# TencentARC/HOSNeRF

Hardware: AMD Instinct MI355X
Metric: train rays/sec (stage3: forward + losses + backward + gradient all-reduce + Adam; LPIPS term OFF in this line -- stages.stage3_with_lpips carries it) (higher is better)
Workload: dtype f32 (fp16/bf16 hi-lo split MFMA x3, fp32 accumulate)

## Files before the change

hosnerf_amd/csrc/hos_compact.hip:

```cpp
#include "hos_common.h"

namespace {

constexpr int CT = 256;
constexpr int CPT = 4;
constexpr int CB = CT * CPT;
constexpr int CMAXB = 4096;

__global__ __launch_bounds__(CT) void compact_count_kernel(const float* mask, float thr, long P, int* blk_off, unsigned int* ticket,
                                                          int* count) {
    __shared__ int sh[CT / 64];
    __shared__ bool last;
    const int tid = threadIdx.x;
    const long base = (long)blockIdx.x * CB + tid * CPT;
    int c = 0;
#pragma unroll
    for (int k = 0; k < CPT; ++k) c += (base + k < P && mask[base + k] > thr) ? 1 : 0;
    for (int o = 32; o > 0; o >>= 1) c += __shfl_xor(c, o, 64);
    if ((tid & 63) == 0) sh[tid >> 6] = c;
    __syncthreads();
    if (tid == 0) {
        int tot = 0;
        for (int w = 0; w < CT / 64; ++w) tot += sh[w];
        blk_off[blockIdx.x] = tot;
// ... 95 lines not shown
__global__ __launch_bounds__(LT) void live_scan_kernel(const int* __restrict__ flag, int B, int S, int* __restrict__ ray_ids,
                                                       int* __restrict__ rows_live) {
    __shared__ int wsum[LT / 64];
    __shared__ int total;
    const int t = threadIdx.x, lane = t & 63, wave = t >> 6;
    const int per = (B + LT - 1) / LT;
    const int r0 = t * per;
    int c = 0;
    for (int k = 0; k < per; ++k) c += (r0 + k < B && flag[r0 + k] != 0) ? 1 : 0;
    int incl = c;
    for (int o = 1; o < 64; o <<= 1) { const int n = __shfl_up(incl, o, 64); if (lane >= o) incl += n; }
    if (lane == 63) wsum[wave] = incl;
    __syncthreads();
    int pos = incl - c;
    for (int w = 0; w < wave; ++w) pos += wsum[w];
    if (t == LT - 1) { total = pos + c; *rows_live = (pos + c) * S; }
    for (int k = 0; k < per; ++k)
        if (r0 + k < B && flag[r0 + k] != 0) ray_ids[pos++] = r0 + k;
    __syncthreads();
    const int n = total;
    for (int i = n + t; i < B; i += LT) ray_ids[i] = -1;
}

__global__ __launch_bounds__(256) void gather_rays_kernel(const float* __restrict__ src, const int* __restrict__ ray_ids,
                                                         const int* __restrict__ rows_live, long P, int S, int C, float* __restrict__ dst) {
    const long total = P * C;
    const long live = min((long)*rows_live, P) * C;
    for (long i = (long)blockIdx.x * blockDim.x + threadIdx.x; i < total; i += (long)gridDim.x * blockDim.x) {
        float v = 0.f;
        if (i < live) {
            const long j = i / C;
            const int c = (int)(i - j * C);
            const long ray = ray_ids[j / S];
            v = src[(ray * S + j % S) * C + c];
        }
        dst[i] = v;
    }
}

__global__ __launch_bounds__(256) void scatter_rays_kernel(const float* __restrict__ src, const int* __restrict__ ray_ids,
                                                          const int* __restrict__ flag, const int* __restrict__ rows_live, long P, int S,
                                                          int C, float* __restrict__ dst) {
    const long total = P * C;
    const long live = min((long)*rows_live, P) * C;
    for (long i = (long)blockIdx.x * blockDim.x + threadIdx.x; i < total; i += (long)gridDim.x * blockDim.x) {
        const long j = i / C;
        const int c = (int)(i - j * C);
        if (i < live) {
            const long ray = ray_ids[j / S];
            dst[(ray * S + j % S) * C + c] = src[i];
        }
        if (flag[j / S] == 0) dst[i] = 0.f;
    }
}

inline int rays_grid(long total) {
    long b = (total + 255) / 256;
    return (int)(b > 4096 ? 4096 : (b < 1 ? 1 : b));
}

}

extern "C" int hos_select_live_rays(const float* mask, float thr, int B, int S, int32_t* ray_ids, int32_t* flag, int32_t* rows_live,
                                    hos_stream_t stream) {
    if (!mask || !ray_ids || !flag || !rows_live || B <= 0 || S <= 0) return HOS_E_ARG;
    if ((long long)B * S > 0x7fffffffLL) return HOS_E_SHAPE;
    hipStream_t s = static_cast<hipStream_t>(stream);
    hipLaunchKernelGGL(live_flag_kernel, dim3((unsigned)((B + 3) / 4)), dim3(256), 0, s, mask, thr, B, S, flag);
    hipLaunchKernelGGL(live_scan_kernel, dim3(1), dim3(LT), 0, s, flag, B, S, ray_ids, rows_live);
    return hos_launch_status();
}

extern "C" int hos_gather_rays(const float* src, const int32_t* ray_ids, const int32_t* rows_live, int B, int S, int C, float* dst,
                               hos_stream_t stream) {
    if (!src || !ray_ids || !rows_live || !dst || B <= 0 || S <= 0 || C <= 0) return HOS_E_ARG;
    const long P = (long)B * S;
    hipLaunchKernelGGL(gather_rays_kernel, dim3(rays_grid(P * C)), dim3(256), 0, static_cast<hipStream_t>(stream), src, ray_ids, rows_live,
                       P, S, C, dst);
    return hos_launch_status();
}

extern "C" int hos_scatter_rays(const float* src, const int32_t* ray_ids, const int32_t* flag, const int32_t* rows_live, int B, int S,
                                int C, float* dst, hos_stream_t stream) {
    if (!src || !ray_ids || !flag || !rows_live || !dst || B <= 0 || S <= 0 || C <= 0) return HOS_E_ARG;
    const long P = (long)B * S;
    hipLaunchKernelGGL(scatter_rays_kernel, dim3(rays_grid(P * C)), dim3(256), 0, static_cast<hipStream_t>(stream), src, ray_ids, flag,
                       rows_live, P, S, C, dst);
    return hos_launch_status();
}

extern "C" long long hos_compact_workspace_ints(void) { return CMAXB + 4; }

extern "C" int hos_compact_rows(const float* mask, float thr, const float* src_a, const float* src_b, int64_t P, int32_t* count,
                                int32_t* sel, float* out_a, float* out_b, int32_t* workspace, hos_stream_t stream) {
    if (!mask || !count || !workspace || P <= 0) return HOS_E_ARG;
    if ((out_a && !src_a) || (out_b && !src_b)) return HOS_E_ARG;
    const long nb = (P + CB - 1) / CB;
    if (nb > CMAXB) return HOS_E_SHAPE;
    hipStream_t s = static_cast<hipStream_t>(stream);
    hipLaunchKernelGGL(compact_count_kernel, dim3((unsigned)nb), dim3(CT), 0, s, mask, thr, (long)P, workspace,
                       reinterpret_cast<unsigned int*>(workspace + CMAXB), count);
    hipLaunchKernelGGL(compact_scatter_kernel, dim3((unsigned)nb), dim3(CT), 0, s, mask, thr, (long)P, workspace, count, src_a, src_b,
                       sel, out_a, out_b);
    return hos_launch_status();
}

extern "C" int hos_scatter_rows(const float* src, const int32_t* sel, const int32_t* count, int64_t P, float* dst, hos_stream_t stream) {
    if (!src || !sel || !count || !dst || P <= 0) return HOS_E_ARG;
    hipStream_t s = static_cast<hipStream_t>(stream);
    {
// ... 8 lines not shown
```

hosnerf_amd/csrc/hos_human.hip:

```cpp
#include "hos_common.h"

constexpr long persist_grid = 768;

namespace {

constexpr int KMAX = 32;

__device__ __forceinline__ float trilinear_zero(const float* __restrict__ vol, int V, float gx, float gy, float gz) {
    const float ix = ((gx + 1.f) / 2.f) * (float)(V - 1);
    const float iy = ((gy + 1.f) / 2.f) * (float)(V - 1);
    const float iz = ((gz + 1.f) / 2.f) * (float)(V - 1);
    const float fx = floorf(ix), fy = floorf(iy), fz = floorf(iz);
    if (!(fx >= -1.f && fx <= (float)V && fy >= -1.f && fy <= (float)V && fz >= -1.f && fz <= (float)V)) return 0.f;
    const int x0 = (int)fx, y0 = (int)fy, z0 = (int)fz;
    const float wx1 = ix - fx, wy1 = iy - fy, wz1 = iz - fz;
    const float wx0 = (fx + 1.f) - ix, wy0 = (fy + 1.f) - iy, wz0 = (fz + 1.f) - iz;
    float out = 0.f;
#pragma unroll
    for (int dz = 0; dz < 2; ++dz)
#pragma unroll
        for (int dy = 0; dy < 2; ++dy)
#pragma unroll
            for (int dx = 0; dx < 2; ++dx) {
                const int x = x0 + dx, y = y0 + dy, z = z0 + dz;
// ... 369 lines not shown
            for (int t = 0; t < 8; ++t) {
                const float v_up = __shfl_up(contrib[t], off, 64);
                if (lane >= off && !flag) contrib[t] += v_up;
            }
            if (lane >= off) flag |= f_up;
        }
        if (act && tail) {
#pragma unroll
            for (int dz = 0; dz < 2; ++dz)
#pragma unroll
                for (int dy = 0; dy < 2; ++dy)
#pragma unroll
                    for (int dx = 0; dx < 2; ++dx) {
                        const int x = x0 + dx, y = y0 + dy, z = z0 + dz;
                        const float cw = contrib[dz * 4 + dy * 2 + dx];
                        if (x >= 0 && x < V && y >= 0 && y < V && z >= 0 && z < V && cw != 0.f)
                            __hip_atomic_fetch_add(g_vol + ((size_t)z * V + y) * V + x, cw, __ATOMIC_RELAXED, __HIP_MEMORY_SCOPE_AGENT);
                    }
        }
    }
    return out;
}

__global__ __launch_bounds__(256) void human_sample_warp_bwd_kernel(
    const float* __restrict__ pts, const float* __restrict__ R, const float* __restrict__ T,
    const float* __restrict__ vol, int V, const float* __restrict__ bbox_min, const float* __restrict__ bbox_scale,
    long P, int K, const float* __restrict__ g_xskel, const float* __restrict__ g_mask,
    float* __restrict__ g_vol, float* __restrict__ g_R, float* __restrict__ g_T, float* __restrict__ aux,
    const float* __restrict__ fwd_xskel, const float* __restrict__ fwd_mask) {
    __shared__ float sR[KMAX * 9], sT[KMAX * 3], sB[6], sAcc[KMAX * 12];
    for (int i = threadIdx.x; i < K * 9; i += blockDim.x) sR[i] = R[i];
    for (int i = threadIdx.x; i < K * 3; i += blockDim.x) sT[i] = T[i];
    for (int i = threadIdx.x; i < K * 12; i += blockDim.x) sAcc[i] = 0.f;
    if (threadIdx.x < 3) { sB[threadIdx.x] = bbox_min[threadIdx.x]; sB[3 + threadIdx.x] = bbox_scale[threadIdx.x]; }
    __syncthreads();
    const long nchunks = (P + 255) / 256;
    for (long chunk = blockIdx.x; chunk < nchunks; chunk += gridDim.x) {
    const long p = chunk * 256 + threadIdx.x;
    const bool live = p < P;
    const long pp = live ? p : P - 1;
    const int lane = threadIdx.x & 63;
    const float px = pts[pp * 3], py = pts[pp * 3 + 1], pz = pts[pp * 3 + 2];
    const size_t V3 = (size_t)V * V * V;
    float wsum, xs, ys, zs;
    if (fwd_xskel != nullptr) {
        wsum = fwd_mask[pp];
        xs = fwd_xskel[pp * 3]; ys = fwd_xskel[pp * 3 + 1]; zs = fwd_xskel[pp * 3 + 2];
    } else {
        float ax = 0.f, ay = 0.f, az = 0.f;
        wsum = 0.f;
        for (int i = 0; i < K; ++i) {
            const float* r = sR + i * 9;
            const float qx = (r[0] * px + r[1] * py + r[2] * pz) + sT[i * 3 + 0];
            const float qy = (r[3] * px + r[4] * py + r[5] * pz) + sT[i * 3 + 1];
            const float qz = (r[6] * px + r[7] * py + r[8] * pz) + sT[i * 3 + 2];
            const float w = trilinear_zero(vol + i * V3, V, (qx - sB[0]) * sB[3] - 1.f, (qy - sB[1]) * sB[4] - 1.f, (qz - sB[2]) * sB[5] - 1.f);
            wsum += w; ax += w * qx; ay += w * qy; az += w * qz;
        }
        const float d0 = fmaxf(wsum, 1e-4f);
        xs = ax / d0; ys = ay / d0; zs = az / d0;
    }
    const float den = fmaxf(wsum, 1e-4f);
    const float clampg = (wsum >= 1e-4f) ? 1.f : 0.f;
// ... 38 lines not shown
                atomicAdd(&sAcc[bone * 12 + comp * 3 + 1], a1);
                atomicAdd(&sAcc[bone * 12 + comp * 3 + 2], a2);
                atomicAdd(&sAcc[bone * 12 + 9 + comp], a3);
            }
        }
        __syncthreads();
    }
    }
    __syncthreads();
    for (int i = threadIdx.x; i < K * 12; i += blockDim.x) {
        const int b = i / 12, c = i % 12;
        const float v = sAcc[i];
        if (v != 0.f) {
            if (c < 9) __hip_atomic_fetch_add(g_R + b * 9 + c, v, __ATOMIC_RELAXED, __HIP_MEMORY_SCOPE_AGENT);
            else __hip_atomic_fetch_add(g_T + b * 3 + (c - 9), v, __ATOMIC_RELAXED, __HIP_MEMORY_SCOPE_AGENT);
        }
    }
}

__global__ __launch_bounds__(1024) void sample_warp_vol_scatter_kernel(
    const float* __restrict__ pts, const float* __restrict__ R, const float* __restrict__ T, int V,
    const float* __restrict__ bbox_min, const float* __restrict__ bbox_scale, long P,
    const float* __restrict__ g_xskel, const float* __restrict__ g_mask, const float* __restrict__ aux,
    float* __restrict__ g_vol) {
    extern __shared__ float s_gvol[];
    const int i = blockIdx.y;
    const int V3 = V * V * V;
    for (int k = threadIdx.x; k < V3; k += blockDim.x) s_gvol[k] = 0.f;
    float r[9], tt[3], bm[3], bs[3];
#pragma unroll
    for (int k = 0; k < 9; ++k) r[k] = R[i * 9 + k];
#pragma unroll
    for (int k = 0; k < 3; ++k) { tt[k] = T[i * 3 + k]; bm[k] = bbox_min[k]; bs[k] = bbox_scale[k]; }
    __syncthreads();
    const int lane = threadIdx.x & 63;
    const long span = (long)gridDim.x * blockDim.x;
    const long p_end = ((P + span - 1) / span) * span;
    for (long p = (long)blockIdx.x * blockDim.x + threadIdx.x; p < p_end; p += span) {
        const bool live = p < P;
        const long pp = live ? p : P - 1;
        const float px = pts[pp * 3], py = pts[pp * 3 + 1], pz = pts[pp * 3 + 2];
        const float qx = (r[0] * px + r[1] * py + r[2] * pz) + tt[0];
        const float qy = (r[3] * px + r[4] * py + r[5] * pz) + tt[1];
        const float qz = (r[6] * px + r[7] * py + r[8] * pz) + tt[2];
        const float gw = ((g_xskel[pp * 3] * qx + g_xskel[pp * 3 + 1] * qy + g_xskel[pp * 3 + 2] * qz) - aux[pp * 2 + 1]) / aux[pp * 2] + g_mask[pp];
        const float gx = (qx - bm[0]) * bs[0] - 1.f, gy = (qy - bm[1]) * bs[1] - 1.f, gz = (qz - bm[2]) * bs[2] - 1.f;
        const float ix = ((gx + 1.f) / 2.f) * (float)(V - 1), iy = ((gy + 1.f) / 2.f) * (float)(V - 1), iz = ((gz + 1.f) / 2.f) * (float)(V - 1);
        const float fx = floorf(ix), fy = floorf(iy), fz = floorf(iz);
        const bool act = live && gw != 0.f && (fx >= -1.f && fx <= (float)V && fy >= -1.f && fy <= (float)V && fz >= -1.f && fz <= (float)V);
        const int x0 = act ? (int)fx : 0, y0 = act ? (int)fy : 0, z0 = act ? (int)fz : 0;
        const float wx1 = ix - fx, wy1 = iy - fy, wz1 = iz - fz;
        const float wx0 = (fx + 1.f) - ix, wy0 = (fy + 1.f) - iy, wz0 = (fz + 1.f) - iz;
        float contrib[8];
#pragma unroll
        for (int t8 = 0; t8 < 8; ++t8) {
            const int dx = t8 & 1, dy = (t8 >> 1) & 1, dz = t8 >> 2;
            contrib[t8] = act ? gw * ((dx ? wx1 : wx0) * (dy ? wy1 : wy0) * (dz ? wz1 : wz0)) : 0.f;
        }
        const int key = act ? ((z0 + 1) * (V + 2) + (y0 + 1)) * (V + 2) + (x0 + 1) : -1 - lane;
        const int key_prev = __shfl_up(key, 1, 64);
        int flag = (lane == 0 || key != key_prev) ? 1 : 0;
        const int key_next = __shfl_down(key, 1, 64);
        const bool tail = (lane == 63) || (key_next != key);
// ... 277 lines not shown
        *reinterpret_cast<float4*>(out + p * ldo + c4 * 4) = o;
    }
}

__global__ __launch_bounds__(256) void slice_pad_kernel(const float* __restrict__ src, int lds, int col0, long P, int width,
                                                        float* __restrict__ out, int ldo, const int* __restrict__ p_dev) {
    if (p_dev) P = min(P, (long)*p_dev);
    const int q = ldo >> 2;
    const long total = P * q;
    for (long it = (long)blockIdx.x * blockDim.x + threadIdx.x; it < total; it += (long)gridDim.x * blockDim.x) {
        const long p = it / q;
        const int c4 = (int)(it % q);
        float v[4] = {0.f, 0.f, 0.f, 0.f};
        if (c4 == 0) {
#pragma unroll
            for (int c = 0; c < 4; ++c) if (c < width) v[c] = src[p * lds + col0 + c];
        }
        *reinterpret_cast<float4*>(out + p * ldo + c4 * 4) = make_float4(v[0], v[1], v[2], v[3]);
    }
}

}

extern "C" int hos_human_sample_warp_bwd(const float* pts, const float* R, const float* T, const float* vol, int V,
                                         const float* bbox_min, const float* bbox_scale, int64_t P, int K,
                                         const float* g_x_skel, const float* g_mask, float* g_vol, float* g_R,
                                         float* g_T, float* scratch, const float* fwd_x_skel, const float* fwd_mask,
                                         hos_stream_t stream) {
    if (!pts || !R || !T || !vol || !bbox_min || !bbox_scale || !g_x_skel || !g_mask || !g_vol || !g_R || !g_T || P <= 0)
        return HOS_E_ARG;
    if (K <= 0 || K > KMAX || V < 2) return HOS_E_SHAPE;
    hipStream_t s = static_cast<hipStream_t>(stream);
    const long sw_chunks = (P + 255) / 256;
    const dim3 grid((unsigned)(sw_chunks < persist_grid ? sw_chunks : persist_grid));
    const size_t vol_bytes = (size_t)V * V * V * sizeof(float);
    const bool split = scratch != nullptr && vol_bytes <= 128 * 1024 && P >= 8192;
    hipLaunchKernelGGL(human_sample_warp_bwd_kernel, grid, dim3(256), 0, s, pts, R, T, vol, V, bbox_min, bbox_scale, (long)P, K,
                       g_x_skel, g_mask, split ? (float*)nullptr : g_vol, g_R, g_T, split ? scratch : (float*)nullptr,
                       (fwd_x_skel && fwd_mask) ? fwd_x_skel : (const float*)nullptr, (fwd_x_skel && fwd_mask) ? fwd_mask : (const float*)nullptr);
    if (split) {
        static bool attr_set = false;
        if (!attr_set) {
            hipError_t e = hipFuncSetAttribute(reinterpret_cast<const void*>(&sample_warp_vol_scatter_kernel),
                                               hipFuncAttributeMaxDynamicSharedMemorySize, 128 * 1024);
            if (e != hipSuccess) return (int)e;
            attr_set = true;
        }
        const int nb = 256 / K > 0 ? 256 / K : 1;
        hipLaunchKernelGGL(sample_warp_vol_scatter_kernel, dim3(nb, K), dim3(1024), vol_bytes, s, pts, R, T, V, bbox_min,
                           bbox_scale, (long)P, g_x_skel, g_mask, scratch, g_vol);
    }
    return hos_launch_status();
}

extern "C" int hos_lbs_forward_bwd(const float* cnl_pts, const float* R_fwd, const float* T_fwd, const float* vol_cl,
                                   int V, int CL, const float* bbox_min, const float* bbox_scale, int64_t P, int K,
                                   const float* g_x_deform, float* g_cnl, float* g_vol_cl, float* g_R, float* g_T,
                                   const int32_t* rows_dev, hos_stream_t stream) {
    if (!cnl_pts || !R_fwd || !T_fwd || !vol_cl || !bbox_min || !bbox_scale || !g_x_deform || !g_R || !g_T || P <= 0)
        return HOS_E_ARG;
    if (K <= 0 || K > KMAX || CL < K || (CL & 3) || V < 2) return HOS_E_SHAPE;
    const long lb_chunks = (P + 255) / 256;
    hipLaunchKernelGGL(lbs_forward_bwd_kernel, dim3((unsigned)(lb_chunks < persist_grid ? lb_chunks : persist_grid)), dim3(256), 0,
                       static_cast<hipStream_t>(stream), cnl_pts, R_fwd, T_fwd, vol_cl, V, CL, bbox_min, bbox_scale,
                       (long)P, K, g_x_deform, g_cnl, g_vol_cl, g_R, g_T, rows_dev);
    return hos_launch_status();
}

static int embed_bwd_launch(const float* x, const float* band_w, int num_freqs, int identity, const float* dA, int lda,
                            int colA, const float* dB, int ldb, int colB, int64_t P, float* g_x, int accumulate,
                            const int32_t* rows_dev, const float* res, hos_stream_t stream);

extern "C" int hos_embed_bwd(const float* x, const float* band_w, int num_freqs, int identity, const float* dA, int lda,
                             int colA, const float* dB, int ldb, int colB, int64_t P, float* g_x, int accumulate,
                             const int32_t* rows_dev, hos_stream_t stream) {
// ... 48 lines not shown
```

hosnerf_amd/human_nerf.py:

```python
from __future__ import annotations

import json
import math
import os
from types import SimpleNamespace
from typing import Dict, List, Optional

import numpy as np
import torch
import torch.nn as nn
import torch.nn.functional as F

from . import ops
from .flat import FlatModule, FlatStore, Region
from .mipnerf360 import select_state, _Lin

SMPL_PARENT = {1: 0, 2: 0, 3: 0, 4: 1, 5: 2, 6: 3, 7: 4, 8: 5, 9: 6, 10: 7, 11: 8, 12: 9, 13: 9, 14: 9, 15: 12,
               16: 13, 17: 14, 18: 16, 19: 17, 20: 18, 21: 19, 22: 20, 23: 21, 24: 23, 25: 22}


class Cfg(dict):

    def __getattr__(self, k):
        try:
# ... 699 lines not shown
            dst_Rs, dst_Ts, cnl_gtfms, motion_weights_priors, dst_posevec=dst_posevec, iter_val=iter_val, **kwargs)
        flow, state, band_w, cond, vol, vol_cl = pro["flow"], pro["state"], pro["band_w"], pro["cond"], pro["vol"], pro["vol_cl"]
        R_b, T_b, R_f, T_f = pro["R_b"], pro["T_b"], pro["R_f"], pro["T_f"]
        if flow:
            R_fp, T_fp, cond_prev = pro["R_fp"], pro["T_fp"], pro["cond_prev"]
        bmin = kwargs["cnl_bbox_min_xyz"].contiguous()
        bscale = kwargs["cnl_bbox_scale_xyz"].contiguous()

        rays_o = rays[0].reshape(-1, 3).float().contiguous()
        rays_d = rays[1].reshape(-1, 3).float().contiguous()
        B = rays_o.shape[0]
        N = cfg.N_samples
        if t_rand is None and cfg.perturb > 0.0:
            t_rand = torch.rand(B, N, device=dev)
        outs: Dict[str, List[torch.Tensor]] = {}
        chunk = int(cfg.chunk)
        live_rays = bool(live_rays and self.stage == 3 and B <= chunk and torch.is_grad_enabled() and ops.thin_dgrad_rows(B * N))
        for c0 in range(0, B, chunk):
            sl = slice(c0, min(B, c0 + chunk))
            tr = None if t_rand is None else t_rand[sl].contiguous()
            grad = torch.is_grad_enabled()
            live = rows_live = None
            if live_rays:
                z, pts, x_skel, mask = ops.human_sample_warp_ad(vol, R_b, T_b, rays_o[sl], rays_d[sl], near[sl].contiguous(),
                                                                far[sl].contiguous(), N, bmin, bscale, tr, K)
                live = ops.select_live_rays(mask.detach().view(-1, N))
                rows_live = live.rows
                x_c = ops.gather_rays(x_skel.reshape(-1, 3), live)
                mask_c = ops.gather_rays(mask.detach().reshape(-1, 1), live).view(-1)
                pts_c = ops.gather_rays(pts.detach().reshape(-1, 3), live)
                cnl = _NonRigidFn.apply(self._token, self, "nr", x_c, cond, band_w, rows_live)
                n_use = 1 + int(flow) + int(with_cycle)
                cnl_uses = list(ops.fanout(cnl, n_use))
                raw = ops.scatter_rays(_CanonicalFn.apply(self._token, self, cnl_uses.pop(), state, rows_live), live)
            elif grad:
                z, pts, x_skel, mask = ops.human_sample_warp_ad(vol, R_b, T_b, rays_o[sl], rays_d[sl], near[sl].contiguous(),
                                                                far[sl].contiguous(), N, bmin, bscale, tr, K)
                cnl = _NonRigidFn.apply(self._token, self, "nr", x_skel, cond, band_w, None)
                n_use = 1 + int(flow) + int(with_cycle)
                cnl_uses = list(ops.fanout(cnl, n_use))
                raw = _CanonicalFn.apply(self._token, self, cnl_uses.pop(), state)
            else:
                z, pts, x_skel, mask = ops.human_sample_warp(rays_o[sl], rays_d[sl], near[sl].contiguous(), far[sl].contiguous(),
                                                             N, R_b, T_b, vol, bmin, bscale, tr, K)
                cnl, _ = self._nonrigid_fwd(self._nr, x_skel, cond, band_w, save=False)
                cnl_uses = [cnl, cnl, cnl]
                raw, _ = self._canonical_fwd(cnl, state, save=False)
            b = z.shape[0]
            if self.stage == 2:
                rgb_map, acc_map, weights, depth_map = ops.raw2outputs(raw.view(b, N, 4), z, rays_d[sl], mask.view(b, N),
                                                                       kwargs["bgcolor"].to(dev))
                ret = {"rgb": rgb_map, "alpha": acc_map, "depth": depth_map, "weights": weights}
            else:
# ... 79 lines not shown
```

hosnerf_amd/ops.py:

```python
from __future__ import annotations

import os
import threading

import math
from typing import Optional, Tuple

import numpy as np
import torch

from . import _lib
from ._lib import call, ptr

EPS = 1.1920929e-07

EPI_NONE, EPI_RELU, EPI_DENSITY, EPI_RGB, EPI_NERF_HEAD, EPI_SIGMOID_RELU4, EPI_RESIDUAL = 0, 1, 2, 3, 4, 5, 6


def round_up(x: int, m: int) -> int:
    return (x + m - 1) // m * m


class KernelEvents:

# ... 1337 lines not shown
    def backward(ctx, g):
        return _scatter_rays_raw(g, ctx.live), None


class _ScatterRays(torch.autograd.Function):
    @staticmethod
    def forward(ctx, src, live):
        ctx.live = live
        return _scatter_rays_raw(src, live)

    @staticmethod
    def backward(ctx, g):
        return _gather_rays_raw(g, ctx.live), None


def gather_rays(src: torch.Tensor, live: LiveRays) -> torch.Tensor:
    return _GatherRays.apply(src, live) if (src.requires_grad and torch.is_grad_enabled()) else _gather_rays_raw(src, live)


def scatter_rays(src: torch.Tensor, live: LiveRays) -> torch.Tensor:
    return _ScatterRays.apply(src, live) if (src.requires_grad and torch.is_grad_enabled()) else _scatter_rays_raw(src, live)


_LOSS_WS = {}


def _loss_workspace(device) -> torch.Tensor:
    key = _stream_key(device)
    if key not in _LOSS_WS:
        _LOSS_WS[key] = torch.zeros(int(_lib.load().hos_train_losses_workspace_floats()), device=device)
    return _LOSS_WS[key]


class _TrainLosses(torch.autograd.Function):

    @staticmethod
    def forward(ctx, rgb, target, mse_const, mse_count, pts_prev, weights, ray_grid, fg, cam, Kin, observe, deform, n_cyc_dev,
                w_mse, w_flow, w_cycle):
        B = rgb.shape[0]
        S = 0 if pts_prev is None else pts_prev.shape[1]
        n_cyc = 0 if observe is None else observe.shape[0]
        out = torch.empty(8, device=rgb.device)
        call("hos_train_losses_fwd", ptr(rgb), ptr(target), B, float(mse_const), float(mse_count), ptr(pts_prev), ptr(weights),
             ptr(ray_grid), ptr(fg, torch.int32), ptr(cam), ptr(Kin), S, ptr(observe), ptr(deform), n_cyc, ptr(n_cyc_dev, torch.int32),
             float(w_mse), float(w_flow), float(w_cycle), ptr(_loss_workspace(rgb.device)), ptr(out))
        ctx.save_for_backward(rgb, target, pts_prev, weights, ray_grid, fg, cam, Kin, observe, deform, n_cyc_dev, out)
# ... 89 lines not shown
                dsts.append(x_out[f])
                g = gs[k]
                srcs.append(None if g is None else g.contiguous())
                k += 1
        copy_or_zero_n(dsts, srcs)
        return tuple(outs)


def unbind_frames_many(*xs):
    F_ = xs[0].shape[0]
    if F_ == 1 or not (torch.is_grad_enabled() and any(x.requires_grad for x in xs)):
        return [tuple(x[f] for f in range(x.shape[0])) for x in xs]
    flat = _UnbindFramesMany.apply(*xs)
    out, k = [], 0
    for x in xs:
        out.append(tuple(flat[k:k + x.shape[0]]))
        k += x.shape[0]
    return out


class _SampleWarp(torch.autograd.Function):

    @staticmethod
    def forward(ctx, vol, R, T, rays_o, rays_d, near, far, N, bmin, bscale, t_rand, K):
        z, pts, x_skel, mask = human_sample_warp(rays_o, rays_d, near, far, N, R, T, vol, bmin, bscale, t_rand, K)
        ctx.save_for_backward(vol, R, T, pts, bmin, bscale, x_skel, mask)
        ctx.K = K
        ctx.mark_non_differentiable(z, pts)
        ctx.set_materialize_grads(False)
        return z, pts, x_skel, mask

    @staticmethod
    def backward(ctx, gz, gpts, g_xskel, g_mask):
        vol, R, T, pts, bmin, bscale, x_skel, mask = ctx.saved_tensors
        K = ctx.K
        P = pts.shape[0] * pts.shape[1]
        g_vol, g_R, g_T = _zeros_like_many(vol, R, T)
        gx = zeros((P, 3), pts.device) if g_xskel is None else g_xskel.contiguous()
        gm = zeros(P, pts.device) if g_mask is None else g_mask.contiguous()
        scratch = torch.empty(P, 2, device=pts.device)
        call("hos_human_sample_warp_bwd", ptr(pts), ptr(R), ptr(T), ptr(vol), vol.shape[-1], ptr(bmin), ptr(bscale), P, K,
             ptr(gx), ptr(gm), ptr(g_vol), ptr(g_R), ptr(g_T), ptr(scratch),
             ptr(x_skel), ptr(mask))
        return g_vol, g_R, g_T, None, None, None, None, None, None, None, None, None


def human_sample_warp_ad(vol, R, T, rays_o, rays_d, near, far, N, bmin, bscale, t_rand=None, K: int = 26):
    return _SampleWarp.apply(vol.contiguous(), R.contiguous(), T.contiguous(), rays_o, rays_d, near, far, N, bmin, bscale, t_rand, K)


class _LbsForward(torch.autograd.Function):
    @staticmethod
    def forward(ctx, cnl, vol_cl, R_f, T_f, bmin, bscale, K, rows_dev):
        out = lbs_forward(cnl, R_f, T_f, vol_cl, bmin, bscale, K, rows_dev)
        ctx.save_for_backward(cnl, vol_cl, R_f, T_f, bmin, bscale, rows_dev)
        ctx.K = K
        return out

    @staticmethod
    def backward(ctx, g):
        cnl, vol_cl, R_f, T_f, bmin, bscale, rows_dev = ctx.saved_tensors
        P = cnl.shape[0]
        g_cnl = torch.empty_like(cnl)
        g_vol, g_R, g_T = _zeros_like_many(vol_cl, R_f, T_f)
        g = g.contiguous()
        call("hos_lbs_forward_bwd", ptr(cnl), ptr(R_f), ptr(T_f), ptr(vol_cl), vol_cl.shape[0], vol_cl.shape[-1], ptr(bmin),
             ptr(bscale), P, ctx.K, ptr(g), ptr(g_cnl), ptr(g_vol), ptr(g_R), ptr(g_T), ptr(rows_dev, torch.int32))
        return g_cnl, g_vol, g_R, g_T, None, None, None, None


def lbs_forward_ad(cnl, vol_cl, R_f, T_f, bmin, bscale, K: int = 26, rows_dev=None):
# ... 176 lines not shown
```

include/hosrender.h:

```cpp
#ifndef HOSRENDER_H
#define HOSRENDER_H

#include <stdint.h>

#ifdef __cplusplus
extern "C" {
#endif

#define HOS_OK 0
#define HOS_E_ARG (-1)
#define HOS_E_ALIGN (-2)
#define HOS_E_SHAPE (-3)
#define HOS_E_NODEVICE (-4)

typedef void* hos_stream_t;

#define HOS_ABI_VERSION 101

int hos_version(void);
int hos_device_count(void);
const char* hos_error_string(int code);


#define HOS_GEMM_MODE_FP32 0
// ... 173 lines not shown
                  float* dz_rgb, int ld_dr, hos_stream_t stream);


int hos_human_sample_warp(const float* rays_o, const float* rays_d, const float* near_, const float* far_,
                          const float* t_vals, const float* t_rand, const float* R, const float* T,
                          const float* vol, int V, const float* bbox_min, const float* bbox_scale,
                          int B, int N, int K, float* z_vals, float* pts, float* x_skel, float* mask,
                          hos_stream_t stream);

int hos_lbs_forward(const float* cnl_pts, const float* R_fwd, const float* T_fwd, const float* vol_cl,
                    int V, int CL, const float* bbox_min, const float* bbox_scale, int64_t P, int K,
                    float* x_deform, const int32_t* rows_dev, hos_stream_t stream);

int hos_embed_hannw(const float* x, const float* band_w, int num_freqs, const float* cond, int cond_size,
                    int64_t P, float* E, int lde, float* PE, int ldpe, const int32_t* rows_dev, hos_stream_t stream);

int hos_embed_fourier(const float* x, int num_freqs, const float* state, int state_size, int64_t P,
                      float* E, int lde, float* E2, int lde2, const int32_t* rows_dev, hos_stream_t stream);

int hos_human_sample_warp_bwd(const float* pts, const float* R, const float* T, const float* vol, int V,
                              const float* bbox_min, const float* bbox_scale, int64_t P, int K,
                              const float* g_x_skel, const float* g_mask, float* g_vol, float* g_R, float* g_T,
                              float* scratch, const float* fwd_x_skel, const float* fwd_mask, hos_stream_t stream);
int hos_lbs_forward_bwd(const float* cnl_pts, const float* R_fwd, const float* T_fwd, const float* vol_cl,
                        int V, int CL, const float* bbox_min, const float* bbox_scale, int64_t P, int K,
                        const float* g_x_deform, float* g_cnl, float* g_vol_cl, float* g_R, float* g_T,
                        const int32_t* rows_dev, hos_stream_t stream);
int hos_embed_bwd(const float* x, const float* band_w, int num_freqs, int identity, const float* dA, int lda,
                  int colA, const float* dB, int ldb, int colB, int64_t P, float* g_x, int accumulate,
                  const int32_t* rows_dev, hos_stream_t stream);
int hos_slice_mask(const float* src, int lds, int col0, const float* mask_src, int ldm, int mcol0, int64_t P,
                   int width, float* out, int ldo, const int32_t* rows_dev, hos_stream_t stream);
int hos_slice_pad(const float* src, int lds, int col0, int64_t P, int width, float* out, int ldo,
                  const int32_t* rows_dev, hos_stream_t stream);
int hos_rgbsigma_grad(const float* g_rgbsigma, const float* rgbsigma, int64_t P, float* dz, int ldz,
                      const int32_t* rows_dev, hos_stream_t stream);

int hos_raw2outputs_fwd(const float* rgbs, int rgb_ld, const float* sigma, int sigma_ld, const float* z_vals,
                        const float* rays_d, const float* mask, const float* bgcolor, float last_dist,
                        int B, int S, float* rgb, float* acc, float* weights, float* depth, hos_stream_t stream);
int hos_raw2outputs_bwd(const float* g_rgb, const float* g_weights, const float* rgbs, int rgb_ld,
                        const float* sigma, int sigma_ld, const float* z_vals, const float* rays_d,
                        const float* mask, const float* bgcolor, float last_dist, int B, int S,
                        float* g_rgbs, int g_rgb_ld, float* g_sigma, int g_sigma_ld, float* g_mask,
                        hos_stream_t stream);

// ... 44 lines not shown
                         const float* aux, float* const* acts6, int ldact, float* xyz, int64_t P,
                         const int32_t* rows_dev, hos_stream_t stream);

int hos_mlp_chain_bwd_steps(int cfg);
long long hos_mlp_chain_bwd_image_bytes(int cfg, int step);
long long hos_mlp_chain_bwd_ws_floats(int cfg, int M);
int hos_mlp_chain_bwd_pack(int n, const int* cfg, const int* step, const float* const* W, const int* ldw, const int* N, const int* K,
                           void* const* image, hos_stream_t stream);
int hos_mlp_chain_bwd(int cfg, const float* dZ, int lddz, int M, const int32_t* rows_dev, const float* const* X, const int* ldx,
                      const void* const* images, float* const* dXout, const int* lddx, float* const* dW, const int* lddw,
                      float* const* db, const int* N, const int* K, float* ws, int64_t ws_floats, hos_stream_t stream);

long long hos_compact_workspace_ints(void);
int hos_compact_rows(const float* mask, float thr, const float* src_a, const float* src_b, int64_t P, int32_t* count,
                     int32_t* sel, float* out_a, float* out_b, int32_t* workspace, hos_stream_t stream);
int hos_scatter_rows(const float* src, const int32_t* sel, const int32_t* count, int64_t P, float* dst, hos_stream_t stream);

int hos_select_live_rays(const float* mask, float thr, int B, int S, int32_t* ray_ids, int32_t* flag, int32_t* rows_live,
                         hos_stream_t stream);
int hos_gather_rays(const float* src, const int32_t* ray_ids, const int32_t* rows_live, int B, int S, int C, float* dst,
                    hos_stream_t stream);
int hos_scatter_rays(const float* src, const int32_t* ray_ids, const int32_t* flag, const int32_t* rows_live, int B, int S,
                     int C, float* dst, hos_stream_t stream);

long long hos_train_losses_workspace_floats(void);
int hos_train_losses_fwd(const float* rgb, const float* target, long long n_rays, float mse_const, float mse_count,
                         const float* pts_prev, const float* weights, const float* ray_grid, const int32_t* fg,
                         const float* cam_prev, const float* intrinsics_prev, int S,
                         const float* observe, const float* deform, long long n_cyc, const int32_t* n_cyc_dev,
                         float w_mse, float w_flow, float w_cycle, float* workspace, float* out8,
                         hos_stream_t stream);
int hos_train_losses_bwd(const float* g_total, const float* out8, const float* rgb, const float* target, long long n_rays,
                         float mse_count, const float* pts_prev, const float* weights, const float* ray_grid,
                         const int32_t* fg, const float* cam_prev, const float* intrinsics_prev, int S,
                         const float* observe, const float* deform, long long n_cyc, const int32_t* n_cyc_dev,
                         float w_mse, float w_flow, float w_cycle,
                         float* g_rgb, float* g_pts_prev, float* g_weights, float* g_deform, hos_stream_t stream);

int hos_sumsq(const float* g, int64_t n, float* sumsq, hos_stream_t stream);
int hos_adam_step(float* p, const float* g, float* m, float* v, int64_t n, float lr, float beta1,
                  float beta2, float eps, int step, float grad_scale, const float* sumsq,
                  float max_norm, hos_stream_t stream);

int hos_adam_step_dyn(float* p, const float* g, float* m, float* v, int64_t n, const float* hyper,
                      float beta1, float beta2, float eps, float grad_scale, const float* sumsq,
                      float max_norm, hos_stream_t stream);
// ... 57 lines not shown
```

Before: 140,700.

## Fuse live-ray gathers and restrict sample-warp backward to live rays

Result: no change. 141,200 (median of 6 runs) (+0.4%).

```diff
diff --git a/hosnerf_amd/csrc/hos_compact.hip b/hosnerf_amd/csrc/hos_compact.hip
--- a/hosnerf_amd/csrc/hos_compact.hip
+++ b/hosnerf_amd/csrc/hos_compact.hip
@@ -141,42 +141,90 @@
     for (int i = n + t; i < B; i += LT) ray_ids[i] = -1;
 }
 
+template <int C> __device__ __forceinline__ void copy_row(const float* __restrict__ src, size_t s, float* __restrict__ dst, size_t d, int Cn) {
+    if (C == 4) {
+        *reinterpret_cast<float4*>(dst + d * 4) = *reinterpret_cast<const float4*>(src + s * 4);
+    } else if (C > 0) {
+        float v[C > 0 ? C : 1];
+#pragma unroll
+        for (int c = 0; c < C; ++c) v[c] = src[s * C + c];
+#pragma unroll
+        for (int c = 0; c < C; ++c) dst[d * C + c] = v[c];
+    } else {
+        for (int c = 0; c < Cn; ++c) dst[d * Cn + c] = src[s * Cn + c];
+    }
+}
+
+template <int C> __device__ __forceinline__ void zero_row(float* __restrict__ dst, size_t d, int Cn) {
+    if (C == 4) {
+        *reinterpret_cast<float4*>(dst + d * 4) = make_float4(0.f, 0.f, 0.f, 0.f);
+    } else if (C > 0) {
+#pragma unroll
+        for (int c = 0; c < C; ++c) dst[d * C + c] = 0.f;
+    } else {
+        for (int c = 0; c < Cn; ++c) dst[d * Cn + c] = 0.f;
+    }
+}
+
+__device__ __forceinline__ long packed_source_row(const int* __restrict__ ray_ids, int j, int B, int S) {
+    const int q = j / S;
+    const int ray = ray_ids[q];
+    return (unsigned)ray < (unsigned)B ? (long)ray * S + (j - q * S) : -1L;
+}
+
+__device__ __forceinline__ int live_rows(const int* __restrict__ rows_live, int P) { return min(max(*rows_live, 0), P); }
+
+template <int C>
 __global__ __launch_bounds__(256) void gather_rays_kernel(const float* __restrict__ src, const int* __restrict__ ray_ids,
-                                                         const int* __restrict__ rows_live, long P, int S, int C, float* __restrict__ dst) {
-    const long total = P * C;
-    const long live = min((long)*rows_live, P) * C;
-    for (long i = (long)blockIdx.x * blockDim.x + threadIdx.x; i < total; i += (long)gridDim.x * blockDim.x) {
-        float v = 0.f;
-        if (i < live) {
-            const long j = i / C;
-            const int c = (int)(i - j * C);
-            const long ray = ray_ids[j / S];
-            v = src[(ray * S + j % S) * C + c];
-        }
-        dst[i] = v;
-    }
-}
-
+                                                         const int* __restrict__ rows_live, int B, int S, int Cn, float* __restrict__ dst) {
+    const int P = B * S;
+    const unsigned ju = blockIdx.x * 256u + threadIdx.x;
+    if (ju >= (unsigned)P) return;
+    const int j = (int)ju;
+    const long r = j < live_rows(rows_live, P) ? packed_source_row(ray_ids, j, B, S) : -1L;
+    if (r >= 0) copy_row<C>(src, (size_t)r, dst, (size_t)j, Cn);
+    else zero_row<C>(dst, (size_t)j, Cn);
+}
+
+template <int C>
 __global__ __launch_bounds__(256) void scatter_rays_kernel(const float* __restrict__ src, const int* __restrict__ ray_ids,
-                                                          const int* __restrict__ flag, const int* __restrict__ rows_live, long P, int S,
-                                                          int C, float* __restrict__ dst) {
-    const long total = P * C;
-    const long live = min((long)*rows_live, P) * C;
-    for (long i = (long)blockIdx.x * blockDim.x + threadIdx.x; i < total; i += (long)gridDim.x * blockDim.x) {
-        const long j = i / C;
-        const int c = (int)(i - j * C);
-        if (i < live) {
-            const long ray = ray_ids[j / S];
-            dst[(ray * S + j % S) * C + c] = src[i];
-        }
-        if (flag[j / S] == 0) dst[i] = 0.f;
-    }
-}
-
-inline int rays_grid(long total) {
-    long b = (total + 255) / 256;
-    return (int)(b > 4096 ? 4096 : (b < 1 ? 1 : b));
-}
+                                                          const int* __restrict__ flag, const int* __restrict__ rows_live, int B, int S,
+                                                          int Cn, float* __restrict__ dst) {
+    const int P = B * S;
+    const unsigned ju = blockIdx.x * 256u + threadIdx.x;
+    if (ju >= (unsigned)P) return;
+    const int j = (int)ju;
+    const int q = j / S;
+    if (j < live_rows(rows_live, P)) {
+        const int ray = ray_ids[q];
+        if ((unsigned)ray < (unsigned)B) copy_row<C>(src, (size_t)j, dst, (size_t)ray * S + (j - q * S), Cn);
+    }
+    if (flag[q] == 0) zero_row<C>(dst, (size_t)j, Cn);
+}
+
+__global__ __launch_bounds__(256) void pack_live_rows_kernel(const float* __restrict__ x_skel, const float* __restrict__ mask,
+                                                            const float* __restrict__ pts, const int* __restrict__ ray_ids,
+                                                            const int* __restrict__ rows_live, int B, int S, float* __restrict__ x_c,
+                                                            float* __restrict__ mask_c, float* __restrict__ pts_c) {
+    const int P = B * S;
+    const unsigned ju = blockIdx.x * 256u + threadIdx.x;
+    if (ju >= (unsigned)P) return;
+    const int j = (int)ju;
+    const long r = j < live_rows(rows_live, P) ? packed_source_row(ray_ids, j, B, S) : -1L;
+    if (r >= 0) {
+        copy_row<3>(x_skel, (size_t)r, x_c, (size_t)j, 3);
+        copy_row<1>(mask, (size_t)r, mask_c, (size_t)j, 1);
+        copy_row<3>(pts, (size_t)r, pts_c, (size_t)j, 3);
+    } else {
+        zero_row<3>(x_c, (size_t)j, 3);
+        zero_row<1>(mask_c, (size_t)j, 1);
+        zero_row<3>(pts_c, (size_t)j, 3);
+    }
+}
+
+inline bool rows_fit_int(int B, int S) { return (long long)B * S <= 0x7fffffffLL; }
+inline unsigned rows_grid(int B, int S) { return (unsigned)(((long)B * S + 255) / 256); }
+inline bool aligned16(const void* a, const void* b) { return ((reinterpret_cast<uintptr_t>(a) | reinterpret_cast<uintptr_t>(b)) & 15) == 0; }
 
 }
 
@@ -193,18 +241,35 @@
 extern "C" int hos_gather_rays(const float* src, const int32_t* ray_ids, const int32_t* rows_live, int B, int S, int C, float* dst,
                                hos_stream_t stream) {
     if (!src || !ray_ids || !rows_live || !dst || B <= 0 || S <= 0 || C <= 0) return HOS_E_ARG;
-    const long P = (long)B * S;
-    hipLaunchKernelGGL(gather_rays_kernel, dim3(rays_grid(P * C)), dim3(256), 0, static_cast<hipStream_t>(stream), src, ray_ids, rows_live,
-                       P, S, C, dst);
+    if (!rows_fit_int(B, S)) return HOS_E_SHAPE;
+    hipStream_t s = static_cast<hipStream_t>(stream);
+    const dim3 grid(rows_grid(B, S)), block(256);
+    if (C == 1) hipLaunchKernelGGL(gather_rays_kernel<1>, grid, block, 0, s, src, ray_ids, rows_live, B, S, C, dst);
+    else if (C == 3) hipLaunchKernelGGL(gather_rays_kernel<3>, grid, block, 0, s, src, ray_ids, rows_live, B, S, C, dst);
+    else if (C == 4 && aligned16(src, dst)) hipLaunchKernelGGL(gather_rays_kernel<4>, grid, block, 0, s, src, ray_ids, rows_live, B, S, C, dst);
+    else hipLaunchKernelGGL(gather_rays_kernel<0>, grid, block, 0, s, src, ray_ids, rows_live, B, S, C, dst);
     return hos_launch_status();
 }
 
 extern "C" int hos_scatter_rays(const float* src, const int32_t* ray_ids, const int32_t* flag, const int32_t* rows_live, int B, int S,
                                 int C, float* dst, hos_stream_t stream) {
     if (!src || !ray_ids || !flag || !rows_live || !dst || B <= 0 || S <= 0 || C <= 0) return HOS_E_ARG;
-    const long P = (long)B * S;
-    hipLaunchKernelGGL(scatter_rays_kernel, dim3(rays_grid(P * C)), dim3(256), 0, static_cast<hipStream_t>(stream), src, ray_ids, flag,
-                       rows_live, P, S, C, dst);
+    if (!rows_fit_int(B, S)) return HOS_E_SHAPE;
+    hipStream_t s = static_cast<hipStream_t>(stream);
+    const dim3 grid(rows_grid(B, S)), block(256);
+    if (C == 1) hipLaunchKernelGGL(scatter_rays_kernel<1>, grid, block, 0, s, src, ray_ids, flag, rows_live, B, S, C, dst);
+    else if (C == 3) hipLaunchKernelGGL(scatter_rays_kernel<3>, grid, block, 0, s, src, ray_ids, flag, rows_live, B, S, C, dst);
+    else if (C == 4 && aligned16(src, dst)) hipLaunchKernelGGL(scatter_rays_kernel<4>, grid, block, 0, s, src, ray_ids, flag, rows_live, B, S, C, dst);
+    else hipLaunchKernelGGL(scatter_rays_kernel<0>, grid, block, 0, s, src, ray_ids, flag, rows_live, B, S, C, dst);
+    return hos_launch_status();
+}
+
+extern "C" int hos_pack_live_rows(const float* x_skel, const float* mask, const float* pts, const int32_t* ray_ids,
+                                  const int32_t* rows_live, int B, int S, float* x_c, float* mask_c, float* pts_c, hos_stream_t stream) {
+    if (!x_skel || !mask || !pts || !ray_ids || !rows_live || !x_c || !mask_c || !pts_c || B <= 0 || S <= 0) return HOS_E_ARG;
+    if (!rows_fit_int(B, S)) return HOS_E_SHAPE;
+    hipLaunchKernelGGL(pack_live_rows_kernel, dim3(rows_grid(B, S)), dim3(256), 0, static_cast<hipStream_t>(stream), x_skel, mask, pts,
+                       ray_ids, rows_live, B, S, x_c, mask_c, pts_c);
     return hos_launch_status();
 }
 
diff --git a/hosnerf_amd/csrc/hos_human.hip b/hosnerf_amd/csrc/hos_human.hip
--- a/hosnerf_amd/csrc/hos_human.hip
+++ b/hosnerf_amd/csrc/hos_human.hip
@@ -415,13 +415,21 @@
     return out;
 }
 
+__device__ __forceinline__ long warp_point(const int* __restrict__ ray_ids, int S, long j) {
+    if (ray_ids == nullptr) return j;
+    const int q = (int)j / S;
+    return (long)max(ray_ids[q], 0) * S + ((int)j - q * S);
+}
+
 __global__ __launch_bounds__(256) void human_sample_warp_bwd_kernel(
     const float* __restrict__ pts, const float* __restrict__ R, const float* __restrict__ T,
     const float* __restrict__ vol, int V, const float* __restrict__ bbox_min, const float* __restrict__ bbox_scale,
     long P, int K, const float* __restrict__ g_xskel, const float* __restrict__ g_mask,
     float* __restrict__ g_vol, float* __restrict__ g_R, float* __restrict__ g_T, float* __restrict__ aux,
-    const float* __restrict__ fwd_xskel, const float* __restrict__ fwd_mask) {
+    const float* __restrict__ fwd_xskel, const float* __restrict__ fwd_mask,
+    const int* __restrict__ ray_ids, const int* __restrict__ rows_live, int S) {
     __shared__ float sR[KMAX * 9], sT[KMAX * 3], sB[6], sAcc[KMAX * 12];
+    if (ray_ids != nullptr) P = min(P, (long)max(*rows_live, 0));
     for (int i = threadIdx.x; i < K * 9; i += blockDim.x) sR[i] = R[i];
     for (int i = threadIdx.x; i < K * 3; i += blockDim.x) sT[i] = T[i];
     for (int i = threadIdx.x; i < K * 12; i += blockDim.x) sAcc[i] = 0.f;
@@ -431,7 +439,7 @@
     for (long chunk = blockIdx.x; chunk < nchunks; chunk += gridDim.x) {
     const long p = chunk * 256 + threadIdx.x;
     const bool live = p < P;
-    const long pp = live ? p : P - 1;
+    const long pp = warp_point(ray_ids, S, live ? p : P - 1);
     const int lane = threadIdx.x & 63;
     const float px = pts[pp * 3], py = pts[pp * 3 + 1], pz = pts[pp * 3 + 2];
     const size_t V3 = (size_t)V * V * V;
@@ -516,8 +524,9 @@
     const float* __restrict__ pts, const float* __restrict__ R, const float* __restrict__ T, int V,
     const float* __restrict__ bbox_min, const float* __restrict__ bbox_scale, long P,
     const float* __restrict__ g_xskel, const float* __restrict__ g_mask, const float* __restrict__ aux,
-    float* __restrict__ g_vol) {
+    float* __restrict__ g_vol, const int* __restrict__ ray_ids, const int* __restrict__ rows_live, int S) {
     extern __shared__ float s_gvol[];
+    if (ray_ids != nullptr) P = min(P, (long)max(*rows_live, 0));
     const int i = blockIdx.y;
     const int V3 = V * V * V;
     for (int k = threadIdx.x; k < V3; k += blockDim.x) s_gvol[k] = 0.f;
@@ -532,7 +541,7 @@
     const long p_end = ((P + span - 1) / span) * span;
     for (long p = (long)blockIdx.x * blockDim.x + threadIdx.x; p < p_end; p += span) {
         const bool live = p < P;
-        const long pp = live ? p : P - 1;
+        const long pp = warp_point(ray_ids, S, live ? p : P - 1);
         const float px = pts[pp * 3], py = pts[pp * 3 + 1], pz = pts[pp * 3 + 2];
         const float qx = (r[0] * px + r[1] * py + r[2] * pz) + tt[0];
         const float qy = (r[3] * px + r[4] * py + r[5] * pz) + tt[1];
@@ -856,11 +865,10 @@
 
 }
 
-extern "C" int hos_human_sample_warp_bwd(const float* pts, const float* R, const float* T, const float* vol, int V,
-                                         const float* bbox_min, const float* bbox_scale, int64_t P, int K,
-                                         const float* g_x_skel, const float* g_mask, float* g_vol, float* g_R,
-                                         float* g_T, float* scratch, const float* fwd_x_skel, const float* fwd_mask,
-                                         hos_stream_t stream) {
+static int sample_warp_bwd_launch(const float* pts, const float* R, const float* T, const float* vol, int V, const float* bbox_min,
+                                  const float* bbox_scale, int64_t P, int K, const float* g_x_skel, const float* g_mask, float* g_vol,
+                                  float* g_R, float* g_T, float* scratch, const float* fwd_x_skel, const float* fwd_mask,
+                                  const int32_t* ray_ids, const int32_t* rows_live, int S, hos_stream_t stream) {
     if (!pts || !R || !T || !vol || !bbox_min || !bbox_scale || !g_x_skel || !g_mask || !g_vol || !g_R || !g_T || P <= 0)
         return HOS_E_ARG;
     if (K <= 0 || K > KMAX || V < 2) return HOS_E_SHAPE;
@@ -871,7 +879,8 @@
     const bool split = scratch != nullptr && vol_bytes <= 128 * 1024 && P >= 8192;
     hipLaunchKernelGGL(human_sample_warp_bwd_kernel, grid, dim3(256), 0, s, pts, R, T, vol, V, bbox_min, bbox_scale, (long)P, K,
                        g_x_skel, g_mask, split ? (float*)nullptr : g_vol, g_R, g_T, split ? scratch : (float*)nullptr,
-                       (fwd_x_skel && fwd_mask) ? fwd_x_skel : (const float*)nullptr, (fwd_x_skel && fwd_mask) ? fwd_mask : (const float*)nullptr);
+                       (fwd_x_skel && fwd_mask) ? fwd_x_skel : (const float*)nullptr, (fwd_x_skel && fwd_mask) ? fwd_mask : (const float*)nullptr,
+                       ray_ids, rows_live, S);
     if (split) {
         static bool attr_set = false;
         if (!attr_set) {
@@ -882,9 +891,29 @@
         }
         const int nb = 256 / K > 0 ? 256 / K : 1;
         hipLaunchKernelGGL(sample_warp_vol_scatter_kernel, dim3(nb, K), dim3(1024), vol_bytes, s, pts, R, T, V, bbox_min,
-                           bbox_scale, (long)P, g_x_skel, g_mask, scratch, g_vol);
+                           bbox_scale, (long)P, g_x_skel, g_mask, scratch, g_vol, ray_ids, rows_live, S);
     }
     return hos_launch_status();
+}
+
+extern "C" int hos_human_sample_warp_bwd(const float* pts, const float* R, const float* T, const float* vol, int V,
+                                         const float* bbox_min, const float* bbox_scale, int64_t P, int K,
+                                         const float* g_x_skel, const float* g_mask, float* g_vol, float* g_R,
+                                         float* g_T, float* scratch, const float* fwd_x_skel, const float* fwd_mask,
+                                         hos_stream_t stream) {
+    return sample_warp_bwd_launch(pts, R, T, vol, V, bbox_min, bbox_scale, P, K, g_x_skel, g_mask, g_vol, g_R, g_T, scratch, fwd_x_skel,
+                                  fwd_mask, nullptr, nullptr, 1, stream);
+}
+
+extern "C" int hos_human_sample_warp_bwd_rays(const float* pts, const float* R, const float* T, const float* vol, int V,
+                                              const float* bbox_min, const float* bbox_scale, int64_t P, int K,
+                                              const float* g_x_skel, const float* g_mask, float* g_vol, float* g_R,
+                                              float* g_T, float* scratch, const float* fwd_x_skel, const float* fwd_mask,
+                                              const int32_t* ray_ids, const int32_t* rows_live, int S, hos_stream_t stream) {
+    if (!ray_ids || !rows_live || S <= 0) return HOS_E_ARG;
+    if (P > 0x7fffffffLL || P % S != 0) return HOS_E_SHAPE;
+    return sample_warp_bwd_launch(pts, R, T, vol, V, bbox_min, bbox_scale, P, K, g_x_skel, g_mask, g_vol, g_R, g_T, scratch, fwd_x_skel,
+                                  fwd_mask, ray_ids, rows_live, S, stream);
 }
 
 extern "C" int hos_lbs_forward_bwd(const float* cnl_pts, const float* R_fwd, const float* T_fwd, const float* vol_cl,
diff --git a/hosnerf_amd/human_nerf.py b/hosnerf_amd/human_nerf.py
--- a/hosnerf_amd/human_nerf.py
+++ b/hosnerf_amd/human_nerf.py
@@ -745,13 +745,12 @@
             grad = torch.is_grad_enabled()
             live = rows_live = None
             if live_rays:
+                holder = ops.LiveRaysHolder()
                 z, pts, x_skel, mask = ops.human_sample_warp_ad(vol, R_b, T_b, rays_o[sl], rays_d[sl], near[sl].contiguous(),
-                                                                far[sl].contiguous(), N, bmin, bscale, tr, K)
-                live = ops.select_live_rays(mask.detach().view(-1, N))
+                                                                far[sl].contiguous(), N, bmin, bscale, tr, K, live_holder=holder)
+                live = holder.live = ops.select_live_rays(mask.detach().view(-1, N))
                 rows_live = live.rows
-                x_c = ops.gather_rays(x_skel.reshape(-1, 3), live)
-                mask_c = ops.gather_rays(mask.detach().reshape(-1, 1), live).view(-1)
-                pts_c = ops.gather_rays(pts.detach().reshape(-1, 3), live)
+                x_c, mask_c, pts_c = ops.pack_live_rows(x_skel.reshape(-1, 3), mask.reshape(-1), pts.reshape(-1, 3), live)
                 cnl = _NonRigidFn.apply(self._token, self, "nr", x_c, cond, band_w, rows_live)
                 n_use = 1 + int(flow) + int(with_cycle)
                 cnl_uses = list(ops.fanout(cnl, n_use))
diff --git a/hosnerf_amd/ops.py b/hosnerf_amd/ops.py
--- a/hosnerf_amd/ops.py
+++ b/hosnerf_amd/ops.py
@@ -1383,6 +1383,43 @@
     return _ScatterRays.apply(src, live) if (src.requires_grad and torch.is_grad_enabled()) else _scatter_rays_raw(src, live)
 
 
+def _pack_live_rows_raw(x_skel, mask, pts, live: LiveRays):
+    P = live.B * live.S
+    x_skel, mask, pts = x_skel.contiguous(), mask.contiguous(), pts.contiguous()
+    dev = x_skel.device
+    x_c, mask_c, pts_c = torch.empty(P, 3, device=dev), torch.empty(P, device=dev), torch.empty(P, 3, device=dev)
+    call("hos_pack_live_rows", ptr(x_skel), ptr(mask), ptr(pts), ptr(live.ray_ids, torch.int32), ptr(live.rows, torch.int32),
+         live.B, live.S, ptr(x_c), ptr(mask_c), ptr(pts_c))
+    return x_c, mask_c, pts_c
+
+
+class _PackLiveRows(torch.autograd.Function):
+    @staticmethod
+    def forward(ctx, x_skel, mask, pts, live):
+        ctx.live = live
+        x_c, mask_c, pts_c = _pack_live_rows_raw(x_skel, mask, pts, live)
+        ctx.mark_non_differentiable(mask_c, pts_c)
+        ctx.set_materialize_grads(False)
+        return x_c, mask_c, pts_c
+
+    @staticmethod
+    def backward(ctx, g_x, g_m, g_p):
+        return (None if g_x is None else _scatter_rays_raw(g_x, ctx.live)), None, None, None
+
+
+def pack_live_rows(x_skel: torch.Tensor, mask: torch.Tensor, pts: torch.Tensor, live: LiveRays):
+    mask, pts = mask.detach(), pts.detach()
+    if x_skel.requires_grad and torch.is_grad_enabled():
+        return _PackLiveRows.apply(x_skel, mask, pts, live)
+    return _pack_live_rows_raw(x_skel, mask, pts, live)
+
+
+class LiveRaysHolder:
+
+    def __init__(self):
+        self.live = None
+
+
 _LOSS_WS = {}
 
 
@@ -1518,8 +1555,9 @@
 class _SampleWarp(torch.autograd.Function):
 
     @staticmethod
-    def forward(ctx, vol, R, T, rays_o, rays_d, near, far, N, bmin, bscale, t_rand, K):
+    def forward(ctx, vol, R, T, rays_o, rays_d, near, far, N, bmin, bscale, t_rand, K, holder):
         z, pts, x_skel, mask = human_sample_warp(rays_o, rays_d, near, far, N, R, T, vol, bmin, bscale, t_rand, K)
+        ctx.holder = holder
         ctx.save_for_backward(vol, R, T, pts, bmin, bscale, x_skel, mask)
         ctx.K = K
         ctx.mark_non_differentiable(z, pts)
@@ -1535,14 +1573,22 @@
         gx = zeros((P, 3), pts.device) if g_xskel is None else g_xskel.contiguous()
         gm = zeros(P, pts.device) if g_mask is None else g_mask.contiguous()
         scratch = torch.empty(P, 2, device=pts.device)
-        call("hos_human_sample_warp_bwd", ptr(pts), ptr(R), ptr(T), ptr(vol), vol.shape[-1], ptr(bmin), ptr(bscale), P, K,
-             ptr(gx), ptr(gm), ptr(g_vol), ptr(g_R), ptr(g_T), ptr(scratch),
-             ptr(x_skel), ptr(mask))
-        return g_vol, g_R, g_T, None, None, None, None, None, None, None, None, None
-
-
-def human_sample_warp_ad(vol, R, T, rays_o, rays_d, near, far, N, bmin, bscale, t_rand=None, K: int = 26):
-    return _SampleWarp.apply(vol.contiguous(), R.contiguous(), T.contiguous(), rays_o, rays_d, near, far, N, bmin, bscale, t_rand, K)
+        live = None if ctx.holder is None else ctx.holder.live
+        if live is not None:
+            assert live.B * live.S == P
+            call("hos_human_sample_warp_bwd_rays", ptr(pts), ptr(R), ptr(T), ptr(vol), vol.shape[-1], ptr(bmin), ptr(bscale), P, K,
+                 ptr(gx), ptr(gm), ptr(g_vol), ptr(g_R), ptr(g_T), ptr(scratch), ptr(x_skel), ptr(mask),
+                 ptr(live.ray_ids, torch.int32), ptr(live.rows, torch.int32), live.S)
+        else:
+            call("hos_human_sample_warp_bwd", ptr(pts), ptr(R), ptr(T), ptr(vol), vol.shape[-1], ptr(bmin), ptr(bscale), P, K,
+                 ptr(gx), ptr(gm), ptr(g_vol), ptr(g_R), ptr(g_T), ptr(scratch),
+                 ptr(x_skel), ptr(mask))
+        return g_vol, g_R, g_T, None, None, None, None, None, None, None, None, None, None
+
+
+def human_sample_warp_ad(vol, R, T, rays_o, rays_d, near, far, N, bmin, bscale, t_rand=None, K: int = 26, live_holder=None):
+    return _SampleWarp.apply(vol.contiguous(), R.contiguous(), T.contiguous(), rays_o, rays_d, near, far, N, bmin, bscale, t_rand, K,
+                             live_holder)
 
 
 class _LbsForward(torch.autograd.Function):
diff --git a/include/hosrender.h b/include/hosrender.h
--- a/include/hosrender.h
+++ b/include/hosrender.h
@@ -219,6 +219,11 @@
                               const float* bbox_min, const float* bbox_scale, int64_t P, int K,
                               const float* g_x_skel, const float* g_mask, float* g_vol, float* g_R, float* g_T,
                               float* scratch, const float* fwd_x_skel, const float* fwd_mask, hos_stream_t stream);
+int hos_human_sample_warp_bwd_rays(const float* pts, const float* R, const float* T, const float* vol, int V,
+                                   const float* bbox_min, const float* bbox_scale, int64_t P, int K,
+                                   const float* g_x_skel, const float* g_mask, float* g_vol, float* g_R, float* g_T,
+                                   float* scratch, const float* fwd_x_skel, const float* fwd_mask, const int32_t* ray_ids,
+                                   const int32_t* rows_live, int S, hos_stream_t stream);
 int hos_lbs_forward_bwd(const float* cnl_pts, const float* R_fwd, const float* T_fwd, const float* vol_cl,
                         int V, int CL, const float* bbox_min, const float* bbox_scale, int64_t P, int K,
                         const float* g_x_deform, float* g_cnl, float* g_vol_cl, float* g_R, float* g_T,
@@ -309,6 +314,8 @@
                     hos_stream_t stream);
 int hos_scatter_rays(const float* src, const int32_t* ray_ids, const int32_t* flag, const int32_t* rows_live, int B, int S,
                      int C, float* dst, hos_stream_t stream);
+int hos_pack_live_rows(const float* x_skel, const float* mask, const float* pts, const int32_t* ray_ids, const int32_t* rows_live,
+                       int B, int S, float* x_c, float* mask_c, float* pts_c, hos_stream_t stream);
 
 long long hos_train_losses_workspace_floats(void);
 int hos_train_losses_fwd(const float* rgb, const float* target, long long n_rays, float mse_const, float mse_count,
```
